# ckonst/VNDecorrelate

Measured on AMD Instinct MI355X. Metric: Msamples/sec decorrelated (stereo, 30 taps) + achieved HBM GB/s vs roofline, higher is better.
Workload: dtype f32

## Files before the change

### vndecorrelate_amd/csrc/vnd_amd.hip

```cpp
#include "vnd_objects.hpp"
#include "vnd_plan.hpp"

extern "C" {


int vnd_abi_version(void) { return VND_ABI_VERSION; }

const char *vnd_last_error(void) { return g_err.c_str(); }

vnd_status vnd_device_count(int32_t *count)
{
    if (!count) return fail(VND_ERR_INVALID, "null count");
    int n = 0;
    hipError_t e = hipGetDeviceCount(&n);
    if (e != hipSuccess) { *count = 0; return fail(VND_ERR_NO_DEVICE, "hipGetDeviceCount: %s", hipGetErrorString(e)); }
    *count = n;
    return VND_OK;
}

vnd_status vnd_ctx_create(int32_t device, vnd_ctx **out)
{
    if (!out) return fail(VND_ERR_INVALID, "null out pointer");
    *out = nullptr;
    int n = 0;
// ... 268 lines not shown

#include "vnd_host.hpp"
#include "vnd_rccl.hpp"

extern "C" {

static vnd_status describe(vnd_ctx *ctx, const vnd_taps *t, int64_t batch, int64_t n, int32_t Cx, int32_t C,
                           int32_t mode, char *text, int32_t len)
{
    vnd_status st = check_shape(ctx, t, batch, n, C, mode, Cx);
    if (st != VND_OK) return st;
    if (!text || len <= 0) return fail(VND_ERR_INVALID, "null text buffer");
    for (int attempt = 0; attempt < 8; ++attempt) {
        const SpecPlan sp = make_spec_plan(ctx, t, nullptr, nullptr, batch, n, C, Cx, mode, nullptr);
        if (!sp.use) break;
        DeviceScope on(ctx->device);
        SpecModule *m = spec_module(ctx, t, sp.cfg, !sp.eager);
        if (m && m->failed && sp.cfg.win && attempt < 7) {
            if (getenv("VND_SPEC_VERBOSE")) fprintf(stderr, "vnd: window form (frames_per_lane=%d threads=%d) unavailable: %s\n", sp.cfg.win, sp.cfg.nt, m->log.c_str());
            continue;
        }
        if (m && !m->failed) {
            if (sp.cfg.win) {
                char split[96];
                if (sp.chunk_tiles > 0) snprintf(split, sizeof split, "a chunk of %d tiles per CU as %d + %d, %d chunks", sp.chunk_tiles, sp.chunk_len0, sp.chunk_tiles - sp.chunk_len0, sp.chunks_per_stream);
                else if (sp.bal_total > 0) snprintf(split, sizeof split, "balanced ranges of %d tiles, %d in the pool", sp.tiles_per_span, sp.bal_total);
                else snprintf(split, sizeof split, "%d spans x %d tiles", sp.spans, sp.tiles_per_span);
                snprintf(text, (size_t)len,
                         "conv_spec%s_window (hipRTC, per table) frames_per_lane=%d tile=%d reads_ahead=%d "
                         "nt_stores=%d mode=%d lds=%zuB workgroups=%u (%u units: %s per stream) threads=%d store_phase=%s%s",
                         sp.cfg.exact ? "_exact" : "", sp.cfg.win, sp.cfg.tile(), sp.cfg.la, sp.cfg.nt_stores, mode,
                         sp.cfg.lds_bytes(), sp.nblocks, sp.units, split, sp.cfg.nt,
                         sp.cfg.win_s ? "planar waves=split-by-channel" : sp.cfg.win_q == 2 ? "planar pieces=channel-octets waves=split-by-channel" : (sp.cfg.win_q ? "planar pieces=channel-quads waves=split-by-channel" : (sp.cfg.win_xpose ? "frame-pairs" : "planar")),
                         sp.cfg.adds ? " taps=adds-per-segment" : "");
                return VND_OK;
            }
            snprintf(text, (size_t)len,
                     "conv_spec%s (hipRTC, per table) pairs_per_lane=%d tile=%d ring_slots=%d prefetch=%d reads_ahead=%d "
                     "nt_stores=%d mode=%d lds=%zuB workgroups=%u (%u units: %d spans x %d tiles per stream) threads=%d",
                     sp.cfg.exact ? "_exact" : "", sp.cfg.rr, sp.cfg.tile(), sp.cfg.pp, sp.cfg.dd, sp.cfg.la, sp.cfg.nt_stores, mode,
                     sp.cfg.lds_bytes(), sp.nblocks, sp.units, sp.spans, sp.tiles_per_span, sp.cfg.nt);
            return VND_OK;
        }
        if (m && getenv("VND_SPEC_VERBOSE")) fprintf(stderr, "vnd: specialised kernel unavailable: %s\n", m->log.c_str());
        break;
    }
    const Plan p = make_plan(ctx, t, batch, n, C, mode, Cx);
    if (p.direct)
        snprintf(text, (size_t)len, "conv_direct mode=%d blocks=%u threads=%d", mode, p.nblocks, kDirectThreads);
    else
        snprintf(text, (size_t)len,
                 "%s%s cg=%d pairs_per_lane=%d tile=%d halo=%d mode=%d lds=%zuB workgroups=%u threads=%d",
                 mode == VND_MODE_FAST ? "conv_fast" : "conv_ordered", p.bc ? "_fanout" : "", p.cg, p.r,
                 2 * p.nt * p.r, p.W - 2 * p.nt * p.r, mode, p.lds_bytes, p.nblocks, p.nt);
    return VND_OK;
}

// ... 43 lines not shown
```

### vndecorrelate_amd/csrc/vnd_hooks.hpp

```cpp
#pragma once

extern "C" {

vnd_status vnd_time_convolve_f32_dev(vnd_ctx *ctx, const vnd_taps *t, const float *x, float *y, int64_t batch,
                                     int64_t n, int32_t C, int32_t mode, int32_t n_buffers, int64_t stride,
                                     int32_t iters, void *stream_, float *avg_ms)
{
    vnd_status st = check_shape(ctx, t, batch, n, C, mode);
    if (st != VND_OK) return st;
    if (!avg_ms || iters <= 0 || n_buffers <= 0) return fail(VND_ERR_INVALID, "bad timing arguments");
    DeviceScope on(ctx->device);
    hipStream_t stream = (hipStream_t)stream_;
    hipEvent_t e0 = nullptr, e1 = nullptr;
    hipError_t he = hipEventCreate(&e0);
    if (he == hipSuccess) he = hipEventCreate(&e1);
    if (he == hipSuccess) he = hipEventRecord(e0, stream);
    for (int i = 0; he == hipSuccess && st == VND_OK && i < iters; ++i) {
        const int64_t off = (int64_t)(i % n_buffers) * stride;
        st = launch(ctx, t, x + off, y + off, batch, n, C, mode, stream);
    }
    float ms = 0.f;
    if (he == hipSuccess) he = hipEventRecord(e1, stream);
    if (he == hipSuccess) he = hipEventSynchronize(e1);
    if (he == hipSuccess) he = hipEventElapsedTime(&ms, e0, e1);
// ... 103 lines not shown
    SpecConfig cfg;
    if (!spec_pick_config(t, tun, 160 * 1024, 0, 0, &cfg, false, false, mode == VND_MODE_EXACT)) return fail(VND_ERR_UNSUPPORTED, "halo does not fit the LDS ring");
    cfg.exact = mode == VND_MODE_EXACT ? 1 : 0;
    return source_out(spec_prologue(t, cfg) + kSpecKernelSource, text, capacity, bytes);
}

vnd_status vnd_window_kernel_source(int32_t C, const int32_t *tap_offsets, const int32_t *tap_index,
                                    const float *tap_weight, const int32_t *seg_offsets, const int32_t *seg_end,
                                    const float *seg_gain, int32_t apply_gain, int32_t mode, int32_t frames_per_lane,
                                    int32_t threads, char *text, int64_t capacity, int64_t *bytes,
                                    int64_t *lds_bytes_per_tile, int64_t *fmas_per_tile)
{
    if (mode != VND_MODE_FAST && mode != VND_MODE_EXACT)
        return fail(VND_ERR_INVALID, "the specialised kernel exists for VND_MODE_FAST and VND_MODE_EXACT");
    if (!bytes) return fail(VND_ERR_INVALID, "null bytes pointer");
    const Tuning tun = tuning_snapshot();
    SpecTable t;
    if (vnd_status st = spec_table_from_csr(C, tap_offsets, tap_index, tap_weight, seg_offsets, seg_end, seg_gain, apply_gain, &t); st != VND_OK)
        return st;
    const int M = frames_per_lane, G = tun.win_g > 0 ? tun.win_g : 8;
    WinGeom g;
    bool quad = C % 8 == 0 && tun.win_quad != 0 && tun.win_octet != 0 && win_geometry(t, M, threads, G, false, 160 * 1024, &g, 2);
    quad = quad || ((C % 4 == 0 || (C % 4 == 2 && C >= 6)) && tun.win_quad != 0 && win_geometry(t, M, threads, G, false, 160 * 1024, &g, 1));
    const bool split = !quad && C == 2 && tun.win_split > 0 && win_geometry(t, M, threads, G, false, 160 * 1024, &g, 0, true);
    const bool bc = C == 2 && tun.win_source_fanout != 0;
    if (bc && !win_geometry(t, M, threads, G, true, 160 * 1024, &g, 0, split))
        return fail(VND_ERR_UNSUPPORTED, "this window geometry does not fit the LDS");
    if (!bc && !quad && !split && !win_geometry(t, M, threads, G, false, 160 * 1024, &g))
        return fail(VND_ERR_UNSUPPORTED, "this window geometry does not fit the LDS");
    SpecConfig cfg = win_config(t, g, tun, mode == VND_MODE_EXACT, bc);
    cfg.epi = (tun.win_source_epi != 0 && !bc && !split && (C == 2 || quad)) ? 1 : 0;
    if (lds_bytes_per_tile || fmas_per_tile) {
        size_t lb = 0, fm = 0;
        if (cfg.exact) win_traffic_exact(t, M, &lb, &fm);
        else win_traffic(t, M, &lb, &fm);
        if (lds_bytes_per_tile) *lds_bytes_per_tile = (int64_t)lb;
        if (fmas_per_tile) *fmas_per_tile = (int64_t)fm;
    }
    return source_out(win_source(t, g, cfg), text, capacity, bytes);
}

vnd_status vnd_code_object_private_bytes(const void *code, int64_t bytes, const char *kernel, int64_t *private_bytes)
{
    if (!code || bytes <= 0 || !kernel || !private_bytes) return fail(VND_ERR_INVALID, "bad arguments");
    const std::vector<char> image((const char *)code, (const char *)code + bytes);
    *private_bytes = spec_private_bytes(image, kernel);
    return VND_OK;
}

// ... 60 lines not shown
```

### vndecorrelate_amd/csrc/vnd_spec.hpp

```cpp
#pragma once
#include <hip/hip_runtime.h>
#include <hip/hiprtc.h>
#include <stdint.h>

#include <sys/stat.h>
#include <sys/types.h>
#include <unistd.h>

#include <algorithm>
#include <cstdarg>
#include <cstring>
#include <cstdio>
#include <cstdlib>
#include <map>
#include <mutex>
#include <string>
#include <tuple>
#include <vector>

namespace vnd {

static const char kSpecKernelSource[] =
#include "vnd_spec_kernel.inc"
    ;

struct SpecConfig {
    int nt = 256;
    int rr = 2;
    int pp = 4;
    int dd = 1;
    int la = 8;
    int nt_stores = 0;
    int exact = 0;
    int epi = 0;
    int bc = 0;
    int shift = 0;
    int win = 0, win_g = 0, win_lds = 0, win_per_cu = 0;
    int win_xpose = 0;
    int win_q = 0;
    int win_s = 0;
    int adds = 0;
    int win_merged = 0;
    int win_late = 0;
    int win_stamps = 0, win_stamp_phases = 0, win_stamp_wave = 0;
    int tile() const { return win ? (win_s ? nt / 2 : (win_q ? nt / (4 * win_q) : nt)) * win : 2 * nt * rr; }
    size_t lds_bytes() const
    {
        if (win) return (size_t)win_lds;
        const size_t pl = (size_t)pp * tile() + 2 * nt + (shift ? 2 : 0);
        return (bc ? 1 : 2) * (shift ? 2 : 1) * pl * 4 + (size_t)2 * (nt / 64) * rr * 2 * 4;
    }
    bool operator<(const SpecConfig &o) const
    {
        return std::tie(nt, rr, pp, dd, la, nt_stores, exact, epi, bc, shift, win, win_g, win_xpose, win_q, win_s, adds, win_merged, win_late,
                        win_stamps, win_stamp_phases, win_stamp_wave) <
               std::tie(o.nt, o.rr, o.pp, o.dd, o.la, o.nt_stores, o.exact, o.epi, o.bc, o.shift, o.win, o.win_g, o.win_xpose, o.win_q, o.win_s,
                        o.adds, o.win_merged, o.win_late, o.win_stamps, o.win_stamp_phases, o.win_stamp_wave);
    }
};

struct SpecTable {
    int C = 0;
    std::vector<int32_t> tap_off;
    std::vector<int32_t> idx;
    std::vector<float> w;
    int max_index = 0;
    std::vector<float> w_raw;
    bool has_seg = false, apply_gain = false;
    std::vector<int32_t> seg_off, seg_end;
    std::vector<float> seg_gain;
};

#define VND_TUNING_VARIABLES(X) \
     \
    X("VND_SPEC_NT", spec_nt, 0) X("VND_SPEC_RR", spec_rr, -1) X("VND_SPEC_DD", spec_dd, -1) X("VND_SPEC_LA", spec_la, -1) \
    X("VND_SPEC_SHIFT", spec_shift, 1) X("VND_WIN_M", win_m, 32) X("VND_WIN_G", win_g, 0) X("VND_WIN_QUAD_M", win_quad_m, 32) \
    X("VND_WIN_SPLIT_LATE", win_split_late, -1) X("VND_WIN_SPLIT_SMALL_NT", win_split_small_nt, 256) \
     \
    X("VND_WIN_EXACT", win_exact, 1) X("VND_WIN_SPLIT_CLASS", win_split_class, 1) X("VND_WIN_QUAD", win_quad, 1) \
    X("VND_WIN_OCTET", win_octet, 1) X("VND_WIN_WIDE", win_wide, 0) X("VND_WIN_SPLIT", win_split, -1) \
    X("VND_WIN_SPLIT_FANOUT", win_split_fanout, 1) X("VND_WIN_FANOUT_EPI", win_fanout_epi, 1) X("VND_WIN_XPOSE_PAIRS", win_xpose_pairs, 1) \
    X("VND_WIN_ADDS", win_adds, 1) X("VND_WIN_EXACT_MERGED", win_exact_merged, 1) \
    X("VND_WIN_SOURCE_FANOUT", win_source_fanout, 0) X("VND_WIN_SOURCE_EPI", win_source_epi, 0) \
    X("VND_EPI_BLOCK_SUMS", epi_block_sums, 1) X("VND_EPI_SUMS_ONLY", epi_sums_only, 1) X("VND_EPI_WIDE", epi_wide, 1) \
    X("VND_EPI_SEQ_SPLIT", epi_seq_split, 1) X("VND_EPI_PAR_COALESCED", epi_par_coalesced, 1) \
     \
    X("VND_WIN_CHUNKS", win_chunks, 1) X("VND_WIN_BALANCE", win_balance, 1) X("VND_WIN_CHUNK_LEN0", win_chunk_len0, 0) \
    X("VND_WIN_STAGGER_TICKS", win_stagger_ticks, 300) X("VND_WIN_PACE", win_pace, 1) X("VND_WIN_PACE_MIN_TILES", win_pace_min_tiles, 16) \
    X("VND_NT_MIN_MB", nt_min_mb, 64) X("VND_NO_NT", no_nt, 0) X("VND_FORCE_NT", force_nt, 0) \
     \
    X("VND_WIN_STAMPS", win_stamps, 0) X("VND_WIN_STAMP_PHASES", win_stamp_phases, 1) X("VND_WIN_STAMP_WAVE", win_stamp_wave, 0)

struct Tuning {
#define VND_TUNING_FIELD(name, field, fallback) int field = fallback;
    VND_TUNING_VARIABLES(VND_TUNING_FIELD)
#undef VND_TUNING_FIELD
};

struct TuningName { const char *name; int Tuning::*field; };
static const TuningName kTuningNames[] = {
// ... 484 lines not shown
```

### vndecorrelate_amd/csrc/vnd_win.hpp

```cpp
#pragma once
#include "vnd_spec.hpp"
#include <cmath>
#include <functional>

namespace vnd {

static const char kWinKernelSource[] =
#include "vnd_win_kernel.inc"
    ;

struct WinGeom {
    int M = 0, nt = 0, G = 8;
    int C = 2;
    int DE = 0;
    int R = 0;
    int NB = 0;
    int plane = 0;
    int npl = 2;
    int tail = 0;
    int quad = 0;
    int split = 0;
    int nh() const { return split ? nt / 2 : (quad ? nt / (4 * quad) : nt); }
    int quad_pad() const { return quad == 2 ? 16 : 0; }
    size_t lds_bytes() const { return (size_t)(quad ? 2 * quad : 1) * (size_t)npl * (size_t)(M / 4) * (size_t)plane + (size_t)quad_pad(); }
    int tile() const { return nh() * M; }
};

inline int win_workgroups_per_cu(const WinGeom &g);

inline bool win_geometry(const SpecTable &t, int M, int nt, int G, bool bc, size_t lds_limit, WinGeom *g, int quad = 0, bool split = false)
{
    if (split && (t.C != 2 || quad || nt % 128 != 0)) return false;
    if (!(M == 16 || M == 32 || M == 64) || nt % 64 != 0 || nt < 64 || nt > 1024 || G < 1) return false;
    if (quad && (quad > 2 || (t.C % (4 * quad) != 0 && !(quad == 1 && t.C % 4 == 2 && t.C >= 6)) || bc || nt % (256 * quad) != 0 || M * quad > 64 || M > 32)) return false;
    if ((int64_t)t.idx.size() * M > 32768) return false;
    if (t.C < 2 || (t.C & 1) || (bc && t.C != 2)) return false;
    g->M = M; g->nt = nt; g->G = G; g->npl = 2; g->C = t.C; g->quad = quad; g->split = split ? 1 : 0;
    const int nh = g->nh();
    const int qc = M / 4;
    auto lay_out = [&](int de, int tail = 0) {
        g->DE = de;
        g->R = nh + g->DE - tail;
        g->tail = tail;
        g->NB = g->DE / G + 1;
        int units = g->R + G + tail;
        const bool swz = qc == 8;
        const int mod_rule = swz ? 4 : std::max(2, 16 / qc), res_rule = swz ? 2 : std::max(1, 8 / qc);
        while (units % mod_rule != res_rule) ++units;
        g->plane = units * 16;
        if ((size_t)(qc - 1) * g->plane + (size_t)G * 16 >= 65536) return false;
        if ((size_t)qc * g->plane >= 65536) return false;
        return g->lds_bytes() <= lds_limit;
    };
    const int de = (t.max_index + M - 1) / M;
    if (!lay_out(de)) return false;
    const int aligned = de + (16 - (nh + de) % 16) % 16;
    if (aligned != de) {
        const int before = win_workgroups_per_cu(*g);
        WinGeom plain = *g;
        if (!(lay_out(aligned) && win_workgroups_per_cu(*g) >= before)) {
            *g = plain;
            const int cut = (nh + de) % 16;
            if (quad && cut > 0 && nh + de - cut >= nh + G && cut <= (nt / 64) * (64 / (M * quad))) {
                if (!(lay_out(de, cut) && win_workgroups_per_cu(*g) >= before)) *g = plain;
            }
        }
    }
    return true;
}

inline int win_waves_per_simd_max(int M, bool split = false) { return split ? (M <= 32 ? 3 : 2) : (M <= 16 ? 3 : (M <= 32 ? 2 : 1)); }

inline int win_workgroups_per_cu(const WinGeom &g)
{
    const int by_lds = (int)std::min<size_t>(std::min<size_t>(16, 2048 / g.nt), (160 * 1024) / g.lds_bytes());
    const int by_regs = std::max(1, win_waves_per_simd_max(g.M, g.split != 0) * 4 / (g.nt / 64));
    return std::max(1, std::min(by_lds, by_regs));
}

struct WinOp { int kind, acc, half; float w; int tap; };
struct WinRead { int ch, o; std::vector<WinOp> ops; };

inline std::vector<WinRead> win_schedule(const SpecTable &t, int ch, int M)
{
    std::vector<std::pair<int, float>> taps;
    for (int32_t k = t.tap_off[ch]; k < t.tap_off[ch + 1]; ++k)
// ... 616 lines not shown
            src += "        }\n    }\n";
        }
        src += "}\n#define VW_TAPS_OF_CHANNEL(pc) vw_taps_of_channel<QD>(pc, b, o);\n#define VW_DISPATCH(pg) switch (pg) {";
        for (int qd = 0; qd < nq; ++qd) spec_append(src, " case %d: vw_span_qc<%d>(a, lds, stream, t_first, ntiles, flags, pace); break;", qd, qd);
        src += " default: break; }\n";
    } else if (g.split) {
        for (int ch = 0; ch < 2; ++ch) src += c.exact ? win_taps_function_exact(t, g, c.la, 0, ch) : win_taps_function(t, g, c.la, 0, ch, c.adds != 0);
        src += "template <int PG> __device__ void vw_taps_of(vw_lchar *const (&b)[2][VW_NBT], float (&o0)[VW_M], float (&o1)[VW_M]);      // (vw_span: not instantiated)\n";
        src += "#define VW_DISPATCH(pg) vw_span_s(a, lds, stream, t_first, ntiles, flags, pace);\n";
    } else {
        const bool merged = c.bc && !c.exact;
        for (int pg = 0; pg < t.C / 2; ++pg) src += c.exact ? (c.win_merged ? win_taps_function_exact_merged(t, g, c.la, pg) : win_taps_function_exact(t, g, c.la, pg)) : (merged ? win_taps_function_merged(t, g, c.la, pg, c.adds != 0) : win_taps_function(t, g, c.la, pg, -1, c.adds != 0));
        src += win_taps_dispatch(t);
    }
    src += fixed.substr(at + marker.size());
    return src;
}

inline SpecConfig win_config(const SpecTable &t, const WinGeom &g, const Tuning &tun, bool exact, bool bc)
{
    SpecConfig c;
    const int M = g.M;
    const bool split = g.split != 0, quad = g.quad != 0;
    c.nt = g.nt; c.win = M; c.win_g = g.G; c.win_lds = (int)g.lds_bytes(); c.win_q = g.quad; c.win_s = g.split;
    c.win_per_cu = win_workgroups_per_cu(g);
    c.rr = 0; c.pp = 0; c.dd = 0;
    c.exact = exact ? 1 : 0; c.bc = bc ? 1 : 0;
    c.la = tun.spec_la >= 0 ? tun.spec_la : ((split && M >= 64) ? (exact ? 3 : 2) : (M >= 32 ? 4 : 6));
    c.win_xpose = (split || quad) ? 0 : (tun.win_xpose_pairs != 0 ? 1 : 0);
    c.adds = (!exact && tun.win_adds != 0 && win_adds_ok(t)) ? 1 : 0;
    c.win_merged = (bc && exact && !split && !quad && tun.win_exact_merged != 0 && win_exact_merged_ok(t)) ? 1 : 0;
    if (split) {
        const int late = M >= 64 ? ((exact && !t.has_seg) ? M / 8 : M / 4 - 1) : 0;
        c.win_late = std::min(std::max(tun.win_split_late >= 0 ? tun.win_split_late : late, 0), M / 4 - 1);
    }
    c.win_stamps = std::min(std::max(tun.win_stamps, 0), 4096);
    c.win_stamp_phases = tun.win_stamp_phases != 0 ? 1 : 0;
    c.win_stamp_wave = std::max(0, tun.win_stamp_wave);
    return c;
}

inline bool win_pick_config(const SpecTable &t, const Tuning &tun, size_t lds_limit, int M, bool small_tiles, bool bc, SpecConfig *out,
                            const std::function<bool(const SpecConfig &)> &rejected, int quad, bool split, bool exact)
{
    static const int kShapes[] = {512, 384, 256, 192, 128, 64};
    const int nt_env = tun.spec_nt, g_env = tun.win_g;
    int best_waves = 0;
    for (int k = 0; k < 6; ++k) {
        const int nt = nt_env > 0 ? nt_env : kShapes[k];
        if (nt_env <= 0 && nt > 256 && quad < 2 && !split) continue;
        if (nt_env <= 0 && nt == 384) continue;
        if (small_tiles && nt_env <= 0 && nt > (quad ? 256 * quad : (split ? tun.win_split_small_nt : 128))) continue;
        for (int G : {8, 4}) {
            if (g_env > 0) G = g_env;
            WinGeom g;
            if (win_geometry(t, M, nt, G, bc, lds_limit, &g, quad, split)) {
                const int waves = win_workgroups_per_cu(g) * (nt / 64);
                if (waves > best_waves) {
                    SpecConfig c = win_config(t, g, tun, exact, bc);
                    if (rejected && rejected(c)) {
                        if (!c.win_xpose) {
                            bool found = false;
                            if (split && M >= 64 && tun.spec_la < 0)
                                while (!found && c.la > 1) { c.la -= 1; found = !rejected(c); }
                            if (!found) continue;
                            best_waves = waves;
                            *out = c;
                            continue;
                        }
                        bool found = false;
                        if (c.la > 3 && tun.spec_la < 0) {
                            c.la -= 1;
                            found = !rejected(c);
                            if (!found) c.la += 1;
                        }
                        if (!found) {
                            c.win_xpose = 0;
                            if (rejected(c)) continue;
                        }
                    }
                    best_waves = waves;
                    *out = c;
                }
            }
            if (g_env > 0) break;
        }
        if (nt_env > 0) break;
    }
    return best_waves > 0;
}

inline std::string win_source_for(const SpecTable &t, const SpecConfig &cfg)
{
    WinGeom g;
    if (!win_geometry(t, cfg.win, cfg.nt, cfg.win_g, cfg.bc != 0, 160 * 1024, &g, cfg.win_q, cfg.win_s != 0)) return "#error window geometry does not fit\n";
    if ((int)g.lds_bytes() != cfg.win_lds) return "#error window geometry changed between the launch plan and the build\n";
    return win_source(t, g, cfg);
}

}
```

### vndecorrelate_amd/csrc/vnd_win_kernel.inc

```
R"VNDWIN(
// vnd_spec_kernel, WINDOW form - the per-table tap sum with a register window (gfx950, wave64).
//
// Compiled at run time with hipRTC (vnd_win.hpp) behind a generated prologue that defines
//   VW_NT   threads per workgroup                 VW_M   consecutive output frames a lane owns per tile (16 | 32 | 64)
//   VW_R    ring entries (one entry = the M frames of one lane's run): NT of the tile + VW_DE of halo
//   VW_G    entries mirrored behind the ring, = the reach of one base register
//   VW_NB   base registers per channel (VW_DE / VW_G + 1)
//   VW_PLANE  bytes between the LDS planes of consecutive 16-byte chunks of an entry
//   VW_LA   LDS reads kept in flight ahead of the FMAs
//   VW_C    interleaved channels of the signal (even): a workgroup takes ONE channel pair of a span, 8 bytes of
//           every VW_C*4-byte frame (VW_C = 2: the whole frame, 16-byte accesses)
//   VW_Q    1: the QUAD form for signals of 4k channels - a workgroup takes a channel QUAD of a span (16 bytes of every
//           frame), a wave computes ONE channel of it (tap functions vw_taps_<pair>c<channel>) and stages and stores whole
//           16-byte pieces for all four (vw_span_qc below)
//           2: the OCTET form for signals of 8k channels - two neighbouring quads (32 bytes of every frame: with 8 channels,
//           whole frames and whole cache lines) per workgroup, an eighth of its lanes per channel
//   VW_S    1: the SPLIT form of a stereo signal - half the workgroup's waves compute channel 0, the others channel 1 (the tap
//           functions vw_taps_c0 / vw_taps_c1): a lane carries one channel's accumulators, so three waves fit a SIMD's registers
//           where the plain form holds two (vw_span_s below)
// and the functions vw_taps(), vw_taps_1(), ... (at the marker below): the tap sum of ONE lane for each channel
// pair, fully unrolled, with vw_taps_of<PG>() to pick one and VW_DISPATCH(pg): the span loop vw_span<pg> of a run-time pair number.
//
// The reference's tap sum (decorrelation.py:649-658, :402-414) asks, per output sample, for one input sample
// per tap.  vnd_spec_kernel.inc reads each of them from LDS (one aligned ds_read_b64 per tap and output
// pair: 4 B per FMA); here a lane owns M CONSECUTIVE outputs of both channels, so the windows
// x[n+i .. n+i+M) of taps whose offsets are closer than M overlap in its registers: the lane reads the
// UNION of its taps' windows once, in ascending 16-byte chunks (ds_read_b128), and every chunk feeds all
// the (tap, output) pairs it covers - 2.6 B per FMA on a 30-tap log-distributed table with M = 32,
// 1.4 B on a uniform 128-tap one.  Tap offsets are compile-time constants, so which register a tap reads
// for which output is static: no address arithmetic, no shuffles.
//   * LDS layout: chunk r of ring entry p lives at r * PLANE + p * 16 (per channel).  Lanes own
//     consecutive entries, so every window read is 64 consecutive 16-byte pieces: conflict-free, and
//     its address is a per-lane base register + an immediate.  The ring wraps at entry granularity:
//     base k holds entry (own + k*G) mod R, the immediate reaches at most G-1 entries further, into
//     the mirror of the ring's first G entries.
//   * arithmetic as in the other fast kernels: v_pk_fma_f32 on aligned pairs.  Even taps accumulate
//     output pairs (0,1), (2,3), ...; odd taps pairs (1,2), (3,4), ... plus outputs 0 and M-1 as single
//     FMAs - everything stays inside the lane, nothing is exchanged between lanes or tiles.  Every
//     output is fl(E + O), E / O = the fma chains over its even / odd taps in ascending offset: the
//     result does not depend on geometry, tile or span position (batch == loop, bit for bit).
//   * no refill region: a tile's own entries die at the barrier that ends its tap phase, and the wave
//     that owned them (a) transposes its outputs through them (planar runs -> interleaved frame
// ... 54 lines not shown
constexpr int VW_NW = VW_NT / 64;
constexpr int VW_QC = VW_M / 4;                 // 16-byte chunks per entry and channel
constexpr int VW_NH = VW_S ? VW_NT / 2 : VW_Q ? VW_NT / (4 * VW_Q) : VW_NT;  // lanes - and ring entries of a tile - per channel pair
constexpr int VW_T = VW_NH * VW_M;              // frames per tile
constexpr int VW_LPE = VW_Q ? VW_M * VW_Q : VW_M / 2;  // lanes of a 1 KB global access that fall into one entry (a lane moves a frame pair; VW_Q: one frame of four channels)
constexpr int VW_EPI_N = 64 / VW_LPE;           // entries per 1 KB global access
constexpr int VW_NI = VW_M / 2;                 // 1 KB global accesses per wave and tile
constexpr int VW_NPL = 2;                       // plane sets in LDS: one per output channel (the store phase transposes both channels' runs through them)
constexpr int VW_NXP = (VW_BC && !VW_S) ? 1 : 2; // ... of them holding INPUT: a mono input is staged once for both outputs (in the split form into both sets)
constexpr int VW_CH = VW_QC * VW_PLANE;         // byte offset of channel 1's planes
constexpr int VW_CX = VW_BC ? 1 : VW_C;         // interleaved INPUT channels
// channel pairs (VW_Q: quads or octets): one per workgroup and span.  4k + 2 channels (6, 10, ...) as QUADS: k full quads and one more that
// starts at channel C - 4 - it overlaps its neighbour in one channel pair, which both workgroups compute and write with the same bits
// (a frame's 16 bytes per access instead of the pair form's 8, for (k + 1) / (k + 1/2) of the arithmetic)
constexpr int VW_PAIRS = VW_Q ? (VW_C + 4 * VW_Q - 1) / (4 * VW_Q) : VW_C / 2;
constexpr int VW_PAIRB = 2 * VW_CH;             // VW_Q: byte offset of the second pair's plane sets
constexpr int VW_QUADB = 2 * VW_PAIRB + VW_QUADPAD; // octets: ... of the second QUAD's (shifted by 16 bytes: the two quads of a frame - neighbouring lanes of the 4-byte staging accesses - in different banks)
static_assert(VW_C >= 2 && VW_C % 2 == 0 && (VW_C == 2 || !VW_BC) && (VW_C == 2 || VW_Q || !VW_EPI), "whole channel pairs; fan-out and fused pointwise steps are stereo (quads / octets: the normaliser's sums only)");
static_assert(VW_Q == 0 || VW_Q == 1 || VW_Q == 2, "pairs, quads or octets");
static_assert(!VW_S || (VW_C == 2 && !VW_Q && !VW_EPI && VW_NT % 128 == 0 && VW_M >= 16), "split form: a stereo table, whole waves per channel");
static_assert(!VW_Q || ((VW_C % (4 * VW_Q) == 0 || (VW_Q == 1 && VW_C % 4 == 2 && VW_C >= 6)) && VW_NT % (256 * VW_Q) == 0 && VW_M * VW_Q <= 64 && VW_M <= 32), "quad / octet form: whole channel quads (4k + 2 channels: the last quad overlaps), whole waves per channel");
static_assert(VW_M == 16 || VW_M == 32 || VW_M == 64, "run length");
constexpr int VW_NBT = VW_NB + VW_TAIL;          // base registers per channel: the ring's, then one per entry offset that reaches into the tail
static_assert(VW_NT % 64 == 0 && VW_R >= VW_NH && VW_R + VW_TAIL == VW_NH + VW_DE && (VW_TAIL == 0 || (VW_Q && VW_R % 16 == 0)), "ring (+ tail) = tile + halo");
static_assert(VW_NB * VW_G > VW_DE, "bases cover the halo");
static_assert((VW_PLANE / 16) >= VW_R + VW_G + VW_TAIL, "plane stride: room for ring + mirror (+ tail)");
static_assert((VW_QC - 1) * VW_PLANE + VW_G * 16 < 65536 && VW_CH < 65536, "ds offset field is 16 bits");
static_assert((VW_Q ? 2 * VW_Q : 1) * VW_NPL * VW_QC * VW_PLANE + VW_QUADPAD <= 160 * 1024 && VW_QUADPAD % 16 == 0, "LDS");

// Raw buffer descriptor (stride 0): num_records = bytes left in the stream, so loads past the end of
// the stream return 0 (the reference's dropped terms, decorrelation.py:656-658) and stores past it
// are discarded.  Built from kernel arguments, blockIdx and the tile counter only: lives in SGPRs.
__device__ __forceinline__ v4i vw_rsrc(const void *base, long long bytes)
{
    const long long cap = 0x7fffffff;
    const unsigned long long addr = (unsigned long long)base;
    v4i r;
    r.x = (int)(unsigned)addr;
    r.y = (int)((unsigned)(addr >> 32) & 0xffffu);
    r.z = (int)(bytes < 0 ? 0 : (bytes > cap ? cap : bytes));
    r.w = 0x00020000;
    return r;
}

// blocks b and b + 8 share an XCD (and its L2): give one XCD consecutive logical ids, so that neighbouring
// spans (whose halos overlap) share an L2
__device__ __forceinline__ unsigned vw_xcd_remap(unsigned b, unsigned nwg)
// ... 611 lines not shown
    const int tl = wl * 64 + ln;                                         // the entry of a tile this LANE computes (in its channel)
    const int we = wl * 64 + pc * 32;                                    // the first of the 32 entries this WAVE stages and stores (both channels)
    const long long f0 = (long long)t_first * VW_T;
    const float *xs = a.x + (stream * a.n + f0) * (XB / 4);
    float *ys = a.y + (stream * a.n + f0) * 2;
    const long long bytes_left = (a.n - f0) * 8;                         // (of the output)
    const long long need = ((long long)ntiles * VW_T + (long long)VW_DE * VW_M) * XB;
    const long long bytes_need = need < (a.n - f0) * XB ? need : (a.n - f0) * XB;
#if VW_LANE_SWIZZLE
    const int lq = (ln & ~24) | ((ln & 8) << 1) | ((ln & 16) >> 1);      // (as vw_span: the 8-byte staging writes and read-backs touch every bank once)
#else
    const int lq = ln;
#endif
    const int lane_e = lq / VW_LPE;
    const int lane_at = ((lq % VW_LPE) >> 1) * VW_PLANE + (lq & 1) * 8;
    // ... and in a 1 KB LOAD: stereo as above; mono - 4 frames = one 16-byte chunk of entry ln / (M / 4), written to both plane sets
    const int in_e = VW_BC ? ln / (VW_M / 4) : lane_e;
    const int in_at = VW_BC ? (ln % (VW_M / 4)) * VW_PLANE : lane_at;
    const int in16 = VW_BC ? ln * 16 : lq * 16;                          // the lane's byte offset in a load
    auto stage = [&](vw_lchar *at, v4f v) {
        if constexpr (VW_BC) { *(vw_lv4f *)at = v; *(vw_lv4f *)(at + VW_CH) = v; }
        else vw_write_pair(at, v);
    };
#if VW_STAMPS && VW_STAMP_PHASES
    const bool vw_stamp_on = blockIdx.x < VW_STAMPS && (a.chunk_tiles > 0 || a.bal_total > 0 || (unsigned)(stream * a.spans + t_first / a.tiles_per_span) == vw_xcd_remap(blockIdx.x, a.nblocks));
    if (vw_stamp_on && threadIdx.x == 0) {
        unsigned hw, xcc;
        asm volatile("s_getreg_b32 %0, hwreg(HW_REG_HW_ID)" : "=s"(hw));
        asm volatile("s_getreg_b32 %0, hwreg(HW_REG_XCC_ID)" : "=s"(xcc));
        vw_stamps[blockIdx.x * 16 + 15] = (unsigned long long)hw | ((unsigned long long)xcc << 32);
    }
#endif
    VW_STAMP_DECL;
    VW_STAMP(0);

    {
        const v4i rx = vw_rsrc(xs, bytes_need);
        constexpr int NFILL = (VW_R + EIN - 1) / EIN;
        constexpr int PER = (NFILL + VW_NW - 1) / VW_NW;
        constexpr int BATCH = 8;
        for (int k0 = 0; k0 < PER; k0 += BATCH) {
            v4f w[BATCH];
#pragma unroll
            for (int kk = 0; kk < BATCH; ++kk) {
                const int i = wv + VW_NW * (k0 + kk);
                w[kk] = vw_load4(rx, i * 1024 + in16, 0, VW_LOAD_AUX);
            }
#pragma unroll
            for (int kk = 0; kk < BATCH; ++kk) {
                const int i = wv + VW_NW * (k0 + kk);
                const int e = i * EIN + in_e;
                if (k0 + kk < PER && e < VW_R) {
                    stage(lds + in_at + e * 16, w[kk]);
                    if (e < VW_G) stage(lds + in_at + (e + VW_R) * 16, w[kk]);
                }
            }
        }
    }
    v4f pre[NE];
    {
        const long long f = ((long long)VW_R + we) * VW_M;
        const v4i rx = vw_rsrc(xs + f * (XB / 4), bytes_need - f * XB);
#pragma unroll
        for (int m = 0; m < NE; ++m) pre[m] = vw_load4(rx, 1024 * m + in16, 0, VW_LOAD_AUX);
    }
    asm volatile("s_waitcnt lgkmcnt(0)\n\ts_barrier" ::: "memory");
    VW_STAMP(1);
    bool hi = (flags & 2) != 0;                                          // (wave-uniform) raised priority: a chunk's first workgroup - or, paced, the one behind
    if (hi) __builtin_amdgcn_s_setprio(2);

    unsigned p0 = 0;
    for (int t = 0; t < ntiles; ++t) {
        // the last tile of the workgroup's last unit refills nothing: no loads, no staging writes, no barrier behind its stores
        const bool fin = (flags & 1) != 0 && t == ntiles - 1;
        const unsigned pw = vw_wrap(p0 + (unsigned)we);
        const unsigned pl = vw_wrap(p0 + (unsigned)tl);
        // (a lane's byte offset in a 1 KB access and its entry in it, made opaque per tile: hipcc otherwise hoists the sums with
        //  64-frame runs is what spilled)
        int lq16 = lq * 16, in16o = in16;
        unsigned pwl = pw + (unsigned)lane_e, pwi = pw + (unsigned)in_e;
        asm volatile("" : "+v"(lq16), "+v"(pwl));
        if constexpr (VW_BC) asm volatile("" : "+v"(in16o), "+v"(pwi));
        float o[VW_M];
        {
            vw_lchar *b[2][VW_NBT];
#pragma unroll
            for (int k = 0; k < VW_NB; ++k) {
                b[0][k] = lds + vw_wrap(pl + (unsigned)(k * VW_G)) * 16u;
                b[1][k] = b[0][k] + VW_CH;
            }
            if (pc == 0) vw_taps_ch<0>(b, o);
            else vw_taps_ch<1>(b, o);
        }
#pragma unroll
        for (int j = 0; j < VW_M; ++j) asm volatile("" : "+v"(o[j]));
        VW_STAMP_TILE(t, 0);
        // X. every wave is done reading this tile's window: the tile's own entries are dead (both channels)
        asm volatile("s_waitcnt lgkmcnt(0)\n\ts_barrier" ::: "memory");
        VW_STAMP_TILE(t, 1);
        if (hi) __builtin_amdgcn_s_setprio(3);
        else __builtin_amdgcn_s_setprio(1);
        // (pacing: the partner's count, in flight through the store phase)
        unsigned seen = 0;
        if (pace.other != nullptr) seen = __hip_atomic_load(pace.other, __ATOMIC_RELAXED, __HIP_MEMORY_SCOPE_AGENT);
        // (the late part of THIS tile's refill: in flight through the transposition and the stores)
        v4f late[LATE > 0 ? LATE : 1];
        if constexpr (LATE > 0) {                                        // (also on a final tile: out of range there, no data moves)
            const long long fl = ((long long)t * VW_NH + VW_R + we) * VW_M;
            const v4i rl = vw_rsrc(xs + fl * (XB / 4), bytes_need - fl * XB);
#pragma unroll
            for (int m = 0; m < LATE; ++m) late[m] = vw_load4(rl, (VW_BC ? in16o : lq16) + 1024 * (NE + m), 0, VW_LOAD_AUX);
        }
        // the lane's run into its own dead entry, planar (its channel's planes)
        vw_lchar *const mine = lds + pc * VW_CH + pl * 16u;
#pragma unroll
        for (int r = 0; r < VW_QC; ++r)
            *(vw_lv4f *)(mine + r * VW_PLANE) = v4f{o[4 * r], o[4 * r + 1], o[4 * r + 2], o[4 * r + 3]};
        // X2. ... and the partner wave's (the other channel of the same 64 entries)
        asm volatile("s_waitcnt lgkmcnt(0)\n\ts_barrier" ::: "memory");
        VW_STAMP_TILE(t, 2);
        const long long fo = (long long)t * VW_T + (long long)we * VW_M;
        const v4i ry = vw_rsrc(ys + fo * 2, bytes_left - fo * 8);
        const long long fi = ((long long)(t + 1) * VW_NH + VW_R + we) * VW_M;
        const v4i rx = vw_rsrc(xs + fi * (XB / 4), bytes_need - fi * XB);
        constexpr int ST_AUX = VW_NT_STORES ? VW_NT_STORE_AUX : 0;
        //  short launch nothing much, covers these round trips: tools/ablate/RUNS.md: run_r4c, run_r4g.sh)
#pragma unroll
        for (int m = 0; m < NI; ++m) {
            vw_lchar *at = lds + lane_at + vw_wrap(pwl + (unsigned)(m * VW_EPI_N)) * 16u;
            const v2f r0 = *(const volatile vw_lv2f *)at, r1 = *(const volatile vw_lv2f *)(at + VW_CH);
            vw_store4(v4f{r0.x, r1.x, r0.y, r1.y}, ry, lq16 + 1024 * m, 0, ST_AUX);
        }
        if (!fin) {
            const bool mirror = pw < (unsigned)VW_G || pw + 32u > (unsigned)VW_R;             // wave-uniform
#pragma unroll
            for (int m = 0; m < NIN; ++m) {
                const unsigned e = vw_wrap((VW_BC ? pwi : pwl) + (unsigned)(m * EIN));
                vw_lchar *at = lds + in_at + e * 16u;
                const v4f v = m < NE ? pre[m < NE ? m : 0] : late[m >= NE ? m - NE : 0];
                stage(at, v);
                if (mirror) { if (e < (unsigned)VW_G) stage(at + VW_R * 16, v); }
                if (m < NE) pre[m < NE ? m : 0] = vw_load4(rx, (VW_BC ? in16o : lq16) + 1024 * m, 0, VW_LOAD_AUX);
            }
        }
        p0 = p0 + VW_NH >= VW_R ? p0 + VW_NH - VW_R : p0 + VW_NH;
        pace.done += 1;
        if (pace.other != nullptr) {
            if (threadIdx.x == 0) __hip_atomic_store(pace.mine, pace.done, __ATOMIC_RELAXED, __HIP_MEMORY_SCOPE_AGENT);
            hi = (unsigned)__builtin_amdgcn_readfirstlane((int)seen) > pace.done;       // the partner is ahead: this workgroup's next tile goes first
        }
        if (hi) __builtin_amdgcn_s_setprio(2);
        else __builtin_amdgcn_s_setprio(0);
        // Y. the refill is in place for every wave's window
        if (!fin) asm volatile("s_waitcnt lgkmcnt(0)\n\ts_barrier" ::: "memory");
        VW_STAMP_TILE(t, 3);
    }
    if (hi) __builtin_amdgcn_s_setprio(0);
    VW_STAMP_FLUSH(vw_stamp_on);
}
#endif

// VW_WAVES_PER_EU: the waves per SIMD that the LDS footprint and the registers let a CU hold - as minimum AND maximum:
// the scheduler must not trade registers for an occupancy the LDS will not grant
extern "C" __global__ __launch_bounds__(VW_NT) __attribute__((amdgpu_waves_per_eu(VW_WAVES_PER_EU, VW_WAVES_PER_EU)))
void vnd_spec_kernel(const VWArgs a)
// ... 77 lines not shown
```

Baseline: 681,300.

## Keep the window's unaligned tail outside the ring in the stereo split form

Extends the ring-plus-tail LDS layout, previously used only by the quad/octet forms, to the stereo split-by-channel window kernel with 64-frame runs. The ring length is rounded to a multiple of 16 entries so waves straddling the ring end stay aligned with the LDS banks. The last few entries live in separate slots behind the mirror, and each tile's refill moves the old tail into the ring and loads the next one. It is on by default for fast mode only when the cut is small, and it adds extra LDS moves, per-tile base-register computation and register pressure.

```diff
diff --git a/vndecorrelate_amd/csrc/vnd_amd.hip b/vndecorrelate_amd/csrc/vnd_amd.hip
--- a/vndecorrelate_amd/csrc/vnd_amd.hip
+++ b/vndecorrelate_amd/csrc/vnd_amd.hip
@@ -314,17 +314,19 @@
         }
         if (m && !m->failed) {
             if (sp.cfg.win) {
-                char split[96];
+                char split[96], ring[32] = "";
+                if (sp.cfg.win_s && sp.cfg.win_tail > 0)
+                    snprintf(ring, sizeof ring, " ring=%d+%d", sp.cfg.nt / 2 + (t->spec_table.max_index + sp.cfg.win - 1) / sp.cfg.win - sp.cfg.win_tail, sp.cfg.win_tail);
                 if (sp.chunk_tiles > 0) snprintf(split, sizeof split, "a chunk of %d tiles per CU as %d + %d, %d chunks", sp.chunk_tiles, sp.chunk_len0, sp.chunk_tiles - sp.chunk_len0, sp.chunks_per_stream);
                 else if (sp.bal_total > 0) snprintf(split, sizeof split, "balanced ranges of %d tiles, %d in the pool", sp.tiles_per_span, sp.bal_total);
                 else snprintf(split, sizeof split, "%d spans x %d tiles", sp.spans, sp.tiles_per_span);
                 snprintf(text, (size_t)len,
                          "conv_spec%s_window (hipRTC, per table) frames_per_lane=%d tile=%d reads_ahead=%d "
-                         "nt_stores=%d mode=%d lds=%zuB workgroups=%u (%u units: %s per stream) threads=%d store_phase=%s%s",
+                         "nt_stores=%d mode=%d lds=%zuB workgroups=%u (%u units: %s per stream) threads=%d store_phase=%s%s%s",
                          sp.cfg.exact ? "_exact" : "", sp.cfg.win, sp.cfg.tile(), sp.cfg.la, sp.cfg.nt_stores, mode,
                          sp.cfg.lds_bytes(), sp.nblocks, sp.units, split, sp.cfg.nt,
                          sp.cfg.win_s ? "planar waves=split-by-channel" : sp.cfg.win_q == 2 ? "planar pieces=channel-octets waves=split-by-channel" : (sp.cfg.win_q ? "planar pieces=channel-quads waves=split-by-channel" : (sp.cfg.win_xpose ? "frame-pairs" : "planar")),
-                         sp.cfg.adds ? " taps=adds-per-segment" : "");
+                         sp.cfg.adds ? " taps=adds-per-segment" : "", ring);
                 return VND_OK;
             }
             snprintf(text, (size_t)len,
diff --git a/vndecorrelate_amd/csrc/vnd_hooks.hpp b/vndecorrelate_amd/csrc/vnd_hooks.hpp
--- a/vndecorrelate_amd/csrc/vnd_hooks.hpp
+++ b/vndecorrelate_amd/csrc/vnd_hooks.hpp
@@ -149,9 +149,9 @@
     WinGeom g;
     bool quad = C % 8 == 0 && tun.win_quad != 0 && tun.win_octet != 0 && win_geometry(t, M, threads, G, false, 160 * 1024, &g, 2);
     quad = quad || ((C % 4 == 0 || (C % 4 == 2 && C >= 6)) && tun.win_quad != 0 && win_geometry(t, M, threads, G, false, 160 * 1024, &g, 1));
-    const bool split = !quad && C == 2 && tun.win_split > 0 && win_geometry(t, M, threads, G, false, 160 * 1024, &g, 0, true);
+    const bool split = !quad && C == 2 && tun.win_split > 0 && win_geometry(t, M, threads, G, false, 160 * 1024, &g, 0, true, win_split_tail_mode(tun, mode == VND_MODE_EXACT));
     const bool bc = C == 2 && tun.win_source_fanout != 0;
-    if (bc && !win_geometry(t, M, threads, G, true, 160 * 1024, &g, 0, split))
+    if (bc && !win_geometry(t, M, threads, G, true, 160 * 1024, &g, 0, split, win_split_tail_mode(tun, mode == VND_MODE_EXACT)))
         return fail(VND_ERR_UNSUPPORTED, "this window geometry does not fit the LDS");
     if (!bc && !quad && !split && !win_geometry(t, M, threads, G, false, 160 * 1024, &g))
         return fail(VND_ERR_UNSUPPORTED, "this window geometry does not fit the LDS");
diff --git a/vndecorrelate_amd/csrc/vnd_spec.hpp b/vndecorrelate_amd/csrc/vnd_spec.hpp
--- a/vndecorrelate_amd/csrc/vnd_spec.hpp
+++ b/vndecorrelate_amd/csrc/vnd_spec.hpp
@@ -41,6 +41,7 @@
     int win_s = 0;
     int adds = 0;
     int win_merged = 0;
+    int win_tail = 0;
     int win_late = 0;
     int win_stamps = 0, win_stamp_phases = 0, win_stamp_wave = 0;
     int tile() const { return win ? (win_s ? nt / 2 : (win_q ? nt / (4 * win_q) : nt)) * win : 2 * nt * rr; }
@@ -52,10 +53,10 @@
     }
     bool operator<(const SpecConfig &o) const
     {
-        return std::tie(nt, rr, pp, dd, la, nt_stores, exact, epi, bc, shift, win, win_g, win_xpose, win_q, win_s, adds, win_merged, win_late,
+        return std::tie(nt, rr, pp, dd, la, nt_stores, exact, epi, bc, shift, win, win_g, win_xpose, win_q, win_s, adds, win_merged, win_late, win_tail,
                         win_stamps, win_stamp_phases, win_stamp_wave) <
                std::tie(o.nt, o.rr, o.pp, o.dd, o.la, o.nt_stores, o.exact, o.epi, o.bc, o.shift, o.win, o.win_g, o.win_xpose, o.win_q, o.win_s,
-                        o.adds, o.win_merged, o.win_late, o.win_stamps, o.win_stamp_phases, o.win_stamp_wave);
+                        o.adds, o.win_merged, o.win_late, o.win_tail, o.win_stamps, o.win_stamp_phases, o.win_stamp_wave);
     }
 };
 
@@ -75,7 +76,7 @@
      \
     X("VND_SPEC_NT", spec_nt, 0) X("VND_SPEC_RR", spec_rr, -1) X("VND_SPEC_DD", spec_dd, -1) X("VND_SPEC_LA", spec_la, -1) \
     X("VND_SPEC_SHIFT", spec_shift, 1) X("VND_WIN_M", win_m, 32) X("VND_WIN_G", win_g, 0) X("VND_WIN_QUAD_M", win_quad_m, 32) \
-    X("VND_WIN_SPLIT_LATE", win_split_late, -1) X("VND_WIN_SPLIT_SMALL_NT", win_split_small_nt, 256) \
+    X("VND_WIN_SPLIT_LATE", win_split_late, -1) X("VND_WIN_SPLIT_TAIL", win_split_tail, 1) X("VND_WIN_SPLIT_SMALL_NT", win_split_small_nt, 256) \
      \
     X("VND_WIN_EXACT", win_exact, 1) X("VND_WIN_SPLIT_CLASS", win_split_class, 1) X("VND_WIN_QUAD", win_quad, 1) \
     X("VND_WIN_OCTET", win_octet, 1) X("VND_WIN_WIDE", win_wide, 0) X("VND_WIN_SPLIT", win_split, -1) \
diff --git a/vndecorrelate_amd/csrc/vnd_win.hpp b/vndecorrelate_amd/csrc/vnd_win.hpp
--- a/vndecorrelate_amd/csrc/vnd_win.hpp
+++ b/vndecorrelate_amd/csrc/vnd_win.hpp
@@ -28,7 +28,10 @@
 
 inline int win_workgroups_per_cu(const WinGeom &g);
 
-inline bool win_geometry(const SpecTable &t, int M, int nt, int G, bool bc, size_t lds_limit, WinGeom *g, int quad = 0, bool split = false)
+constexpr int kSplitTailPays = 4;
+inline int win_split_tail_mode(const Tuning &tun, bool exact) { return tun.win_split_tail == 1 ? (exact ? 0 : 1) : (tun.win_split_tail > 1 ? 2 : 0); }
+
+inline bool win_geometry(const SpecTable &t, int M, int nt, int G, bool bc, size_t lds_limit, WinGeom *g, int quad = 0, bool split = false, int split_tail = 2)
 {
     if (split && (t.C != 2 || quad || nt % 128 != 0)) return false;
     if (!(M == 16 || M == 32 || M == 64) || nt % 64 != 0 || nt < 64 || nt > 1024 || G < 1) return false;
@@ -62,6 +65,9 @@
             *g = plain;
             const int cut = (nh + de) % 16;
             if (quad && cut > 0 && nh + de - cut >= nh + G && cut <= (nt / 64) * (64 / (M * quad))) {
+                if (!(lay_out(de, cut) && win_workgroups_per_cu(*g) >= before)) *g = plain;
+            }
+            if (split && split_tail > 0 && M == 64 && cut > 0 && (split_tail > 1 || cut <= kSplitTailPays) && nh + de - cut >= nh + G) {
                 if (!(lay_out(de, cut) && win_workgroups_per_cu(*g) >= before)) *g = plain;
             }
         }
@@ -724,7 +730,7 @@
     SpecConfig c;
     const int M = g.M;
     const bool split = g.split != 0, quad = g.quad != 0;
-    c.nt = g.nt; c.win = M; c.win_g = g.G; c.win_lds = (int)g.lds_bytes(); c.win_q = g.quad; c.win_s = g.split;
+    c.nt = g.nt; c.win = M; c.win_g = g.G; c.win_lds = (int)g.lds_bytes(); c.win_q = g.quad; c.win_s = g.split; c.win_tail = split ? g.tail : 0;
     c.win_per_cu = win_workgroups_per_cu(g);
     c.rr = 0; c.pp = 0; c.dd = 0;
     c.exact = exact ? 1 : 0; c.bc = bc ? 1 : 0;
@@ -756,7 +762,7 @@
         for (int G : {8, 4}) {
             if (g_env > 0) G = g_env;
             WinGeom g;
-            if (win_geometry(t, M, nt, G, bc, lds_limit, &g, quad, split)) {
+            if (win_geometry(t, M, nt, G, bc, lds_limit, &g, quad, split, win_split_tail_mode(tun, exact))) {
                 const int waves = win_workgroups_per_cu(g) * (nt / 64);
                 if (waves > best_waves) {
                     SpecConfig c = win_config(t, g, tun, exact, bc);
@@ -795,7 +801,7 @@
 inline std::string win_source_for(const SpecTable &t, const SpecConfig &cfg)
 {
     WinGeom g;
-    if (!win_geometry(t, cfg.win, cfg.nt, cfg.win_g, cfg.bc != 0, 160 * 1024, &g, cfg.win_q, cfg.win_s != 0)) return "#error window geometry does not fit\n";
+    if (!win_geometry(t, cfg.win, cfg.nt, cfg.win_g, cfg.bc != 0, 160 * 1024, &g, cfg.win_q, cfg.win_s != 0, cfg.win_tail > 0 ? 2 : 0)) return "#error window geometry does not fit\n";
     if ((int)g.lds_bytes() != cfg.win_lds) return "#error window geometry changed between the launch plan and the build\n";
     return win_source(t, g, cfg);
 }
diff --git a/vndecorrelate_amd/csrc/vnd_win_kernel.inc b/vndecorrelate_amd/csrc/vnd_win_kernel.inc
--- a/vndecorrelate_amd/csrc/vnd_win_kernel.inc
+++ b/vndecorrelate_amd/csrc/vnd_win_kernel.inc
@@ -18,6 +18,9 @@
 //   VW_S    1: the SPLIT form of a stereo signal - half the workgroup's waves compute channel 0, the others channel 1 (the tap
 //           functions vw_taps_c0 / vw_taps_c1): a lane carries one channel's accumulators, so three waves fit a SIMD's registers
 //           where the plain form holds two (vw_span_s below)
+//   VW_TAIL entries of the window kept OUTSIDE the ring, behind its mirror, so that VW_R is a multiple of 16 entries and a wave that
+//           straddles the ring's end stays in step with the LDS banks (VW_R + VW_TAIL = tile + halo): quads / octets, and the split
+//           form with 64-frame runs; 0: the whole window in the ring
 // and the functions vw_taps(), vw_taps_1(), ... (at the marker below): the tap sum of ONE lane for each channel
 // pair, fully unrolled, with vw_taps_of<PG>() to pick one and VW_DISPATCH(pg): the span loop vw_span<pg> of a run-time pair number.
 //
@@ -118,7 +121,7 @@
 static_assert(!VW_Q || ((VW_C % (4 * VW_Q) == 0 || (VW_Q == 1 && VW_C % 4 == 2 && VW_C >= 6)) && VW_NT % (256 * VW_Q) == 0 && VW_M * VW_Q <= 64 && VW_M <= 32), "quad / octet form: whole channel quads (4k + 2 channels: the last quad overlaps), whole waves per channel");
 static_assert(VW_M == 16 || VW_M == 32 || VW_M == 64, "run length");
 constexpr int VW_NBT = VW_NB + VW_TAIL;          // base registers per channel: the ring's, then one per entry offset that reaches into the tail
-static_assert(VW_NT % 64 == 0 && VW_R >= VW_NH && VW_R + VW_TAIL == VW_NH + VW_DE && (VW_TAIL == 0 || (VW_Q && VW_R % 16 == 0)), "ring (+ tail) = tile + halo");
+static_assert(VW_NT % 64 == 0 && VW_R >= VW_NH && VW_R + VW_TAIL == VW_NH + VW_DE && (VW_TAIL == 0 || ((VW_Q || (VW_S && VW_TAIL < 16)) && VW_R % 16 == 0)), "ring (+ tail) = tile + halo");
 static_assert(VW_NB * VW_G > VW_DE, "bases cover the halo");
 static_assert((VW_PLANE / 16) >= VW_R + VW_G + VW_TAIL, "plane stride: room for ring + mirror (+ tail)");
 static_assert((VW_QC - 1) * VW_PLANE + VW_G * 16 < 65536 && VW_CH < 65536, "ds offset field is 16 bits");
@@ -776,6 +779,14 @@
         if constexpr (VW_BC) { *(vw_lv4f *)at = v; *(vw_lv4f *)(at + VW_CH) = v; }
         else vw_write_pair(at, v);
     };
+    // The TAIL (VW_TAIL > 0): the window's last VW_TAIL entries, past the ring's 16-aligned length, in slots of their own behind the
+    // mirror.  With the ring holding entries [t, t + R) and the tail [t + R, t + R + TAIL), the refill of a tile's NH dead entries
+    // STARTS with the old tail: the wave that owns the tile's first entries (we == 0) moves those inside the LDS, and the lanes of its
+    // refill accesses that would have loaded them load the NEXT tail instead - NH entries further down the stream, same descriptor -
+    // and stage it into the tail's slots.  All of it wave-private and in LDS program order: the same NH new entries per tile and
+    // channel from memory, the same three barriers.  tail_lane(m, ie): access m's lane (entry ie of the access) is such a lane.
+    constexpr int TOFF = VW_NH * VW_M * XB;                              // byte offset of the next tail from the entry it replaces
+    auto tail_lane = [&](int m, int ie) -> bool { return VW_TAIL > 0 && m * EIN < VW_TAIL && we == 0 && m * EIN + ie < VW_TAIL; };
 #if VW_STAMPS && VW_STAMP_PHASES
     const bool vw_stamp_on = blockIdx.x < VW_STAMPS && (a.chunk_tiles > 0 || a.bal_total > 0 || (unsigned)(stream * a.spans + t_first / a.tiles_per_span) == vw_xcd_remap(blockIdx.x, a.nblocks));
     if (vw_stamp_on && threadIdx.x == 0) {
@@ -790,7 +801,7 @@
 
     {
         const v4i rx = vw_rsrc(xs, bytes_need);
-        constexpr int NFILL = (VW_R + EIN - 1) / EIN;
+        constexpr int NFILL = (VW_R + VW_TAIL + EIN - 1) / EIN;      // (the tail's entries follow the ring's in the stream)
         constexpr int PER = (NFILL + VW_NW - 1) / VW_NW;
         constexpr int BATCH = 8;
         for (int k0 = 0; k0 < PER; k0 += BATCH) {
@@ -804,8 +815,8 @@
             for (int kk = 0; kk < BATCH; ++kk) {
                 const int i = wv + VW_NW * (k0 + kk);
                 const int e = i * EIN + in_e;
-                if (k0 + kk < PER && e < VW_R) {
-                    stage(lds + in_at + e * 16, w[kk]);
+                if (k0 + kk < PER && e < VW_R + VW_TAIL) {
+                    stage(lds + in_at + (e < VW_R ? e : e + VW_G) * 16, w[kk]);      // ring slot e, or tail slot behind the mirror
                     if (e < VW_G) stage(lds + in_at + (e + VW_R) * 16, w[kk]);
                 }
             }
@@ -816,7 +827,7 @@
         const long long f = ((long long)VW_R + we) * VW_M;
         const v4i rx = vw_rsrc(xs + f * (XB / 4), bytes_need - f * XB);
 #pragma unroll
-        for (int m = 0; m < NE; ++m) pre[m] = vw_load4(rx, 1024 * m + in16, 0, VW_LOAD_AUX);
+        for (int m = 0; m < NE; ++m) pre[m] = vw_load4(rx, 1024 * m + in16 + (tail_lane(m, in_e) ? TOFF : 0), 0, VW_LOAD_AUX);
     }
     asm volatile("s_waitcnt lgkmcnt(0)\n\ts_barrier" ::: "memory");
     VW_STAMP(1);
@@ -843,6 +854,19 @@
                 b[0][k] = lds + vw_wrap(pl + (unsigned)(k * VW_G)) * 16u;
                 b[1][k] = b[0][k] + VW_CH;
             }
+#if VW_TAIL
+            // entry offsets VW_R - VW_NH + 1 ... VW_DE: in the ring for the tile's first lanes, in the tail for its last ones.  The fast
+            // mode reads far-first: these bases serve the tile's first reads and die (tlo opaque per tile: not hoisted out of the loop)
+            unsigned tlo = (unsigned)tl;
+            asm volatile("" : "+v"(tlo));
+#pragma unroll
+            for (int j = 0; j < VW_TAIL; ++j) {
+                const unsigned d = (unsigned)(VW_R - VW_NH + 1 + j);
+                const unsigned e = tlo + d;                                                  // entry of the tile's window
+                b[0][VW_NB + j] = lds + (e < (unsigned)VW_R ? vw_wrap(pl + d) : e + (unsigned)VW_G) * 16u;
+                b[1][VW_NB + j] = b[0][VW_NB + j] + VW_CH;
+            }
+#endif
             if (pc == 0) vw_taps_ch<0>(b, o);
             else vw_taps_ch<1>(b, o);
         }
@@ -857,13 +881,14 @@
         // (pacing: the partner's count, in flight through the store phase)
         unsigned seen = 0;
         if (pace.other != nullptr) seen = __hip_atomic_load(pace.other, __ATOMIC_RELAXED, __HIP_MEMORY_SCOPE_AGENT);
+        const int ine = VW_BC ? in16o / (4 * VW_M) : lq16 / (16 * VW_LPE);                 // (in_e, from the opaque offsets: tail_lane's compares belong to this phase)
         // (the late part of THIS tile's refill: in flight through the transposition and the stores)
         v4f late[LATE > 0 ? LATE : 1];
         if constexpr (LATE > 0) {                                        // (also on a final tile: out of range there, no data moves)
             const long long fl = ((long long)t * VW_NH + VW_R + we) * VW_M;
             const v4i rl = vw_rsrc(xs + fl * (XB / 4), bytes_need - fl * XB);
 #pragma unroll
-            for (int m = 0; m < LATE; ++m) late[m] = vw_load4(rl, (VW_BC ? in16o : lq16) + 1024 * (NE + m), 0, VW_LOAD_AUX);
+            for (int m = 0; m < LATE; ++m) late[m] = vw_load4(rl, (VW_BC ? in16o : lq16) + 1024 * (NE + m) + (tail_lane(NE + m, ine) ? TOFF : 0), 0, VW_LOAD_AUX);
         }
         // the lane's run into its own dead entry, planar (its channel's planes)
         vw_lchar *const mine = lds + pc * VW_CH + pl * 16u;
@@ -886,15 +911,39 @@
             vw_store4(v4f{r0.x, r1.x, r0.y, r1.y}, ry, lq16 + 1024 * m, 0, ST_AUX);
         }
         if (!fin) {
+#if VW_TAIL
+            // the old tail is what the tile's first VW_TAIL dead entries become (p0 is a multiple of 16: no wrap inside them): moved by
+            // the wave that has just read its outputs back from them, 16 bytes per lane and step, BEFORE its lanes overwrite the tail
+            if (we == 0) {                                                               // wave-uniform
+                constexpr int NMV = (VW_TAIL * 2 * VW_QC + 63) / 64;                   // steps: 64 pieces of 16 bytes each
+                int lno = ln;
+                asm volatile("" : "+v"(lno));
+                // (a lane's piece: plane set and chunk, of EPM entries per step; one step at a time and no lane masked - lanes past an odd
+                //  tail's end move its last entry once more, the same bytes to the same place: the masked form, all reads first, cost the
+                //  fast form of cfg3's table 16 registers and cfg2's its place under 240)
+                constexpr int EPM = 64 / (2 * VW_QC);
+                static_assert(EPM >= 1, "a 16-byte piece per lane");
+                vw_lchar *const piece = lds + ((lno / VW_QC) & 1) * VW_CH + (lno % VW_QC) * VW_PLANE;
+#pragma unroll
+                for (int i = 0; i < NMV; ++i) {
+                    const int e0 = i * EPM + lno / (2 * VW_QC);
+                    const int el = e0 < VW_TAIL ? e0 : VW_TAIL - 1;
+                    const v4f mv = *(const volatile vw_lv4f *)(piece + (VW_R + VW_G + el) * 16);
+                    vw_lchar *at = piece + (p0 + (unsigned)el) * 16u;
+                    *(vw_lv4f *)at = mv;
+                    if (p0 == 0u) { if (el < VW_G) *(vw_lv4f *)(at + VW_R * 16) = mv; }
+                }
+            }
+#endif
             const bool mirror = pw < (unsigned)VW_G || pw + 32u > (unsigned)VW_R;             // wave-uniform
 #pragma unroll
             for (int m = 0; m < NIN; ++m) {
-                const unsigned e = vw_wrap((VW_BC ? pwi : pwl) + (unsigned)(m * EIN));
+                const unsigned e = tail_lane(m, ine) ? (unsigned)(VW_R + VW_G + m * EIN) + (unsigned)ine : vw_wrap((VW_BC ? pwi : pwl) + (unsigned)(m * EIN));
                 vw_lchar *at = lds + in_at + e * 16u;
                 const v4f v = m < NE ? pre[m < NE ? m : 0] : late[m >= NE ? m - NE : 0];
                 stage(at, v);
                 if (mirror) { if (e < (unsigned)VW_G) stage(at + VW_R * 16, v); }
-                if (m < NE) pre[m < NE ? m : 0] = vw_load4(rx, (VW_BC ? in16o : lq16) + 1024 * m, 0, VW_LOAD_AUX);
+                if (m < NE) pre[m < NE ? m : 0] = vw_load4(rx, (VW_BC ? in16o : lq16) + 1024 * m + (tail_lane(m, ine) ? TOFF : 0), 0, VW_LOAD_AUX);
             }
         }
         p0 = p0 + VW_NH >= VW_R ? p0 + VW_NH - VW_R : p0 + VW_NH;
```

Measured after the change: 679,900. No clear change (-0.2%).
